# ZhangYuef/Alink

Hardware: AMD Instinct MI355X
Metric: rows/sec/node + iters-to-converge, KMeans k=100 1e8-row×128-dim at 1/2/4/8 MI355X (higher is better)
Workload: dtype bf16

## Files before the change

alink_amd/ops/csrc/kmeans_v10.hip:

```cpp
#include <hip/hip_runtime.h>
#include <stdint.h>
#include <stdlib.h>

#ifndef KM10_TIMING
#define KM10_TIMING 0
#endif

#ifndef KM10_PFD
#define KM10_PFD 0
#endif

#include "kmeans_tile.h"
#include "kmeans_v10_body.h"

namespace {

using namespace kmtile;

typedef float f32x32 __attribute__((ext_vector_type(32)));
typedef float f32x16 __attribute__((ext_vector_type(16)));
typedef float f32x4v __attribute__((ext_vector_type(4)));
typedef uint32_t u32x4 __attribute__((ext_vector_type(4)));

enum Mode10 { FULL = 0, LOAD_ONLY = 1, COMPUTE_ONLY = 2, DIST_ONLY = 3, ACC_ONLY = 4 };

constexpr int NBUF = 9;
constexpr int AHEAD = 7;
constexpr int OFF_ASG = NBUF * TILE;
constexpr uint32_t IDX_MODE = 0xC000u;
constexpr int OFF_CNT = OFF_ASG + 512;
constexpr int OFF_DYN = OFF_CNT + 128 * 4;
constexpr int OFF_JUNK = OFF_DYN + 8 * 4;
constexpr int LDS_BYTES = OFF_JUNK + 256;
constexpr int CH = 16;
constexpr int RED_STRIDE = 112 * D;
static_assert(LDS_BYTES <= LDS_CAP && 2 * RED_STRIDE * 4 <= NBUF * TILE, "LDS plan");


__device__ __forceinline__ float max3_raw(float a, float b, float c) {
    float r;
    asm("v_max3_f32 %0, %1, %2, %3" : "=v"(r) : "v"(a), "v"(b), "v"(c));
    return r;
}
__device__ __forceinline__ float max_raw(float a, float b) {
    float r;
    asm("v_max_f32 %0, %1, %2" : "=v"(r) : "v"(a), "v"(b));
    return r;
}

template <int NT>
__device__ __forceinline__ void dma_tile(uint32_t m0v, uint32_t voff, __amdgpu_buffer_rsrc_t rs, uint32_t soff) {
    uint32_t keep, m1, s1, s2, s3;
#define KM10_DMA(POL)                                                                                       \
    asm volatile(                                                                                           \
        "s_mov_b32 %0, m0\n\t"                                                                              \
        "s_mov_b32 m0, %7\n\t"                                                                              \
        "s_add_u32 %2, %8, 4096\n\t"                                                                        \
        "buffer_load_dwordx4 %5, %6, %8 offen " POL " lds\n\t"                                              \
        "s_add_u32 %1, %7, 4096\n\t"                                                                        \
        "s_mov_b32 m0, %1\n\t"                                                                              \
        "s_add_u32 %3, %8, 8192\n\t"                                                                        \
        "buffer_load_dwordx4 %5, %6, %2 offen " POL " lds\n\t"                                              \
        "s_add_u32 %1, %7, 8192\n\t"                                                                        \
        "s_mov_b32 m0, %1\n\t"                                                                              \
        "s_add_u32 %4, %8, 12288\n\t"                                                                       \
        "buffer_load_dwordx4 %5, %6, %3 offen " POL " lds\n\t"                                              \
        "s_add_u32 %1, %7, 12288\n\t"                                                                       \
        "s_mov_b32 m0, %1\n\t"                                                                              \
        "s_nop 0\n\t"                                                                                       \
        "buffer_load_dwordx4 %5, %6, %4 offen " POL " lds\n\t"                                              \
        "s_mov_b32 m0, %0"                                                                                  \
        : "=&s"(keep), "=&s"(m1), "=&s"(s1), "=&s"(s2), "=&s"(s3)                                           \
        : "v"(voff), "s"(rs), "s"(m0v), "s"(soff)                                                           \
        : "memory")
    if constexpr (NT) KM10_DMA("nt");
    else KM10_DMA("");
#undef KM10_DMA
}

__device__ __forceinline__ void l2_touch(uint32_t m0v, uint32_t voff, __amdgpu_buffer_rsrc_t rs, uint32_t soff) {
    uint32_t keep;
    asm volatile(
        "s_mov_b32 %0, m0\n\t"
        "s_mov_b32 m0, %3\n\t"
        "s_nop 0\n\t"
        "buffer_load_dword %1, %2, %4 offen lds\n\t"
        "s_mov_b32 m0, %0"
        : "=&s"(keep)
        : "v"(voff), "s"(rs), "s"(m0v), "s"(soff)
        : "memory");
}

template <int KB, int MODE, int NT, int DYN>
__global__ __launch_bounds__(512) void kmeans_v10_kernel(const __bf16* __restrict__ Xp, int64_t N,
                                                         const __bf16* __restrict__ Cp,
                                                         const float* __restrict__ ninit, float* __restrict__ slab,
                                                         float* __restrict__ slab_cnt, int* __restrict__ assign_out,
                                                         int64_t ntiles, int64_t per, int rev,
                                                         unsigned* __restrict__ dyn_ctr, int dyn_par, int nqs,
                                                         int64_t pool_base, int npool,
                                                         const unsigned* __restrict__ skip, int pfd_arg) {
    static_assert(KB >= 1 && KB <= 7, "v10 holds at most 112 centroids in registers");
    const int pfd = KM10_PFD ? pfd_arg : 0;
    constexpr bool LOADS = MODE == FULL || MODE == LOAD_ONLY;
    __shared__ __attribute__((aligned(1024))) char lds[LDS_BYTES];
    if (skip != nullptr && __hip_atomic_load(skip, __ATOMIC_RELAXED, __HIP_MEMORY_SCOPE_AGENT) != 0u) return;
    const int tid = threadIdx.x;
    const int lane = tid & 63;
    const int wave = __builtin_amdgcn_readfirstlane(tid >> 6);
    const int g = lane >> 4;
    const int li = lane & 15;
    const int64_t tbase = (int64_t)blockIdx.x * per;
    const int nt = (int)(ntiles > tbase ? (ntiles - tbase < per ? ntiles - tbase : per) : 0);
    const int np = (nt + 1) >> 1;
    const int ntp = 2 * np;
    const uint32_t lbase = (uint32_t)(uintptr_t)(LDS_AS void*)lds;
#if KM10_TIMING
    int64_t* const stamp = reinterpret_cast<int64_t*>(assign_out) + 16 * (int64_t)blockIdx.x;
    if (tid == 0) stamp[0] = (int64_t)__builtin_amdgcn_s_memrealtime();
    assign_out = nullptr;
#endif
    auto phys = [&](int t) { return rev ? ntp - 1 - t : t; };
    int* const dstate = reinterpret_cast<int*>(lds + OFF_DYN);
    int* const qbase = dstate + 4;
    auto dphys = [&](int t) -> int64_t {
        const int q = t / CH, o = t % CH;
        if (q < nqs) {
            const int qq = rev ? nqs - 1 - q : q;
            return ((int64_t)blockIdx.x * nqs + qq) * CH + (rev ? CH - 1 - o : o);
        }
        return (int64_t)qbase[q & 3] + o;
    };

    const bool dma_wave = wave >= 4;
    const int prow = (tid & 255) >> 4;
    const uint32_t voff = (uint32_t)(prow * ROWB + (((tid & 15)) ^ xsw(prow)) * 16);
    const int64_t rem_rows = N - tbase * TR;
    const int64_t region = rem_rows * ROWB < (int64_t)nt * TILE ? rem_rows * ROWB : (int64_t)nt * TILE;
    const __amdgpu_buffer_rsrc_t rs = __builtin_amdgcn_make_buffer_rsrc(
        (void*)(reinterpret_cast<const char*>(Xp) + tbase * TILE), (short)0, (int)(region > 0 ? region : 0),
        0x00020000);
    const uint32_t m0_wave = lbase + (uint32_t)((wave - 4) * 1024);
    const uint32_t pf_off = (uint32_t)((wave - 4) * 4096 + lane * 64);
    uint32_t stage_slot = 0;
    auto next_slot = [](uint32_t s) { return s == (uint32_t)((NBUF - 1) * TILE) ? 0u : s + (uint32_t)TILE; };
    auto stage_tile = [&](int t) {
        if constexpr (DYN) {
            const int64_t pt = __builtin_amdgcn_readfirstlane((int)dphys(t));
            const int64_t remb = (N - pt * TR) * ROWB;
            const __amdgpu_buffer_rsrc_t rt = __builtin_amdgcn_make_buffer_rsrc(
                (void*)(reinterpret_cast<const char*>(Xp) + pt * TILE), (short)0,
                (int)(remb <= 0 ? 0 : (remb < TILE ? remb : TILE)), 0x00020000);
            dma_tile<NT>(__builtin_amdgcn_readfirstlane(m0_wave + (uint32_t)(t % NBUF) * TILE), voff, rt, 0u);
        } else {
            dma_tile<NT>(__builtin_amdgcn_readfirstlane(m0_wave + stage_slot), voff, rs,
                         __builtin_amdgcn_readfirstlane((uint32_t)phys(t) * TILE));
            stage_slot = next_slot(stage_slot);
            if (pfd > 0) {
                const int pt = t + pfd < ntp ? t + pfd : ntp - 1;
                l2_touch(lbase + OFF_JUNK, pf_off, rs, __builtin_amdgcn_readfirstlane((uint32_t)phys(pt) * TILE));
            }
        }
    };
    int last_staged = -1;
    if constexpr (DYN) {
        if (tid == 0) {
            if (blockIdx.x == 0) dyn_ctr[dyn_par ^ 1] = 0u;
            int nq = nqs, done = npool <= 0;
            while (!done && nq * CH < AHEAD) {
                const unsigned r = __hip_atomic_fetch_add(dyn_ctr + dyn_par, 1u, __ATOMIC_RELAXED,
                                                          __HIP_MEMORY_SCOPE_AGENT);
                if ((int)r < npool) {
                    qbase[nq & 3] = (int)(pool_base + (int64_t)(rev ? npool - 1 - (int)r : (int)r) * CH);
                    ++nq;
                } else {
                    done = 1;
                }
            }
            dstate[0] = nq;
            dstate[1] = done;
        }
        __syncthreads();
        if (LOADS && dma_wave) {
            const int known = dstate[0] * CH;
            for (int s = 0; s < AHEAD; ++s)
                if (s < known) {
                    stage_tile(s);
                    last_staged = s;
                }
        }
    } else {
        if (LOADS && dma_wave)
            for (int s = 0; s < AHEAD - 2; ++s)
                if (s < ntp) stage_tile(s);
    }
    uint32_t* cnt = reinterpret_cast<uint32_t*>(lds + OFF_CNT);
    if (tid < 128) cnt[tid] = 0u;
    if (tid < 128) reinterpret_cast<uint32_t*>(lds + OFF_ASG)[tid] = IDX_MODE | (IDX_MODE << 16);
#if KM10_TIMING
    uint64_t wait_vm_cyc = 0, wait_bar_cyc = 0;
#endif
    int np_dyn = 0x3fffffff;
    auto read_state = [&](int j) {
        const int nq = dstate[2 * (j & 1)], done = dstate[2 * (j & 1) + 1];
        np_dyn = done ? nq * CH / 2 : 0x3fffffff;
        return nq;
    };

    auto pre = [&](int j) {
        if constexpr (DYN) {
            if (LOADS && dma_wave) {
                const int younger = last_staged - (2 * j + 1);
                if (younger >= 3) wait_vm<12>();
                else if (younger == 2) wait_vm<8>();
                else if (younger == 1) wait_vm<4>();
                else wait_vm<0>();
            }
            barrier_lds();
            const int known = read_state(j) * CH;
            if (LOADS && dma_wave) {
                if (2 * j + AHEAD - 2 < known) {
                    stage_tile(2 * j + AHEAD - 2);
                    last_staged = 2 * j + AHEAD - 2;
                }
                if (2 * j + AHEAD - 1 < known) {
                    stage_tile(2 * j + AHEAD - 1);
                    last_staged = 2 * j + AHEAD - 1;
                }
            }
            return;
        }
#if KM10_TIMING
        const uint64_t tw0 = __builtin_readcyclecounter();
#endif
        if (LOADS && dma_wave && j < np) {
            const int issued = 2 * j + AHEAD - 3 < ntp - 1 ? 2 * j + AHEAD - 3 : ntp - 1;
            const int younger = issued - (2 * j + 1);
            if (pfd > 0) {
                if (younger >= 3) wait_vm<16>();
                else if (younger == 2) wait_vm<11>();
                else if (younger == 1) wait_vm<6>();
                else wait_vm<1>();
            } else {
                wait_tile_np<4, 3>(younger);
            }
        }
#if KM10_TIMING
        const uint64_t tw1 = __builtin_readcyclecounter();
#endif
        barrier_lds();
#if KM10_TIMING
        wait_vm_cyc += tw1 - tw0;
        wait_bar_cyc += __builtin_readcyclecounter() - tw1;
#endif
        if (LOADS && dma_wave) {
            if (2 * j + AHEAD - 2 < ntp) stage_tile(2 * j + AHEAD - 2);
            if (2 * j + AHEAD - 1 < ntp) stage_tile(2 * j + AHEAD - 1);
        }
    };

    if (wave < 4) {
        const int myrow = 16 * wave + li;
        const int apos = 16 * ((myrow >> 2) & 3) + 4 * (myrow >> 4) + (myrow & 3);
        bf16x8 cf[KB][4];
        f32x4 nin[KB];
#pragma unroll
        for (int b = 0; b < KB; ++b) {
#pragma unroll
            for (int s = 0; s < 4; ++s)
                cf[b][s] = *reinterpret_cast<const bf16x8*>(Cp + (16 * b + li) * D + 8 * (s + 4 * g));
            nin[b] = *reinterpret_cast<const f32x4*>(ninit + 16 * b + 4 * g);
        }
        int xr[4];
#pragma unroll
        for (int s = 0; s < 4; ++s) xr[s] = xoff(myrow, s + 4 * g);
        auto load_frag = [&](uint32_t slot, bf16x8 (&x)[4]) {
            const char* xt = lds + slot;
#pragma unroll
            for (int s = 0; s < 4; ++s) x[s] = *reinterpret_cast<const bf16x8*>(xt + xr[s]);
        };
        auto cross_max = [&](float run) {
            const uint32_t u = __float_as_uint(run);
            const auto p32 = __builtin_amdgcn_permlane32_swap(u, u, false, false);
            const uint32_t u2 = __float_as_uint(max_raw(__uint_as_float(p32[0]), __uint_as_float(p32[1])));
            const auto p16 = __builtin_amdgcn_permlane16_swap(u2, u2, false, false);
            return __float_as_uint(max_raw(__uint_as_float(p16[0]), __uint_as_float(p16[1])));
        };
        uint32_t keepmask;
        asm volatile("v_mov_b32 %0, 0xffffff80" : "=v"(keepmask));
        const uint32_t g4 = 4u * (uint32_t)g;
        auto packs = [&](float v, uint32_t field) { return __uint_as_float((__float_as_uint(v) & keepmask) | field); };
        auto rare_neg = [&](const bf16x8 (&x)[4], uint32_t u, uint32_t c) {
            float run = -3.4e38f;
#pragma unroll
            for (int b = 0; b < KB; ++b) {
                f32x4 acc = nin[b];
#pragma unroll
                for (int s = 0; s < 4; ++s) acc = __builtin_amdgcn_mfma_f32_16x16x32_bf16(cf[b][s], x[s], acc, 0, 0, 0);
                const uint32_t c0 = (uint32_t)(16 * b);
                run = max3_raw(run, packs(acc[0], c0), packs(acc[1], c0 + 1));
                run = max3_raw(run, packs(acc[2], c0 + 2), packs(acc[3], c0 + 3));
            }
            const uint32_t v = cross_max(__uint_as_float(__float_as_uint(run) + g4));
            return (int32_t)u < 0 ? (v & 127u) : c;
        };
        auto pair_max = [&](const bf16x8 (&xa_)[4], const bf16x8 (&xb_)[4], uint32_t& ca, uint32_t& cb) {
            f32x4 acc[2 * KB];
            float run[2] = {-3.4e38f, -3.4e38f};
            float p0 = 0.f, p1 = 0.f, p2 = 0.f, p3 = 0.f;
            uint32_t uA = 0u, w0 = 0u, w1 = 0u;
            auto seam = [&](int i) {
                if (i == 0) {
                    uA = __float_as_uint(run[0]) - g4;
                    const auto p32 = __builtin_amdgcn_permlane32_swap(uA, uA, false, false);
                    w0 = p32[0];
                    w1 = p32[1];
                } else if (i == 1) {
                    const uint32_t u2 = __float_as_uint(max_raw(__uint_as_float(w0), __uint_as_float(w1)));
                    const auto p16 = __builtin_amdgcn_permlane16_swap(u2, u2, false, false);
                    w0 = p16[0];
                    w1 = p16[1];
                } else {
                    uA = __float_as_uint(max_raw(__uint_as_float(w0), __uint_as_float(w1)));
                }
            };
#pragma unroll
            for (int t = 0; t < 2 * KB + 2; ++t) {
                const bool mf = t < 2 * KB, vl = t >= 2;
                const int b = t < KB ? t : t - KB;
                const int pt = (t - 2) / KB, pb = (t - 2) % KB;
                const uint32_t f0 = 127u - (uint32_t)(16 * pb);
                auto mfma = [&](int s) {
                    if (!mf) return;
                    acc[t] = __builtin_amdgcn_mfma_f32_16x16x32_bf16(cf[b][s], t < KB ? xa_[s] : xb_[s],
                                                                     s == 0 ? nin[b] : acc[t], 0, 0, 0);
                };
                mfma(0);
                if (vl) {
                    p0 = packs(acc[t - 2][0], f0);
                    p1 = packs(acc[t - 2][1], f0 - 1);
                }
                __builtin_amdgcn_sched_barrier(0);
                mfma(1);
                if (vl) {
                    run[pt] = max3_raw(run[pt], p0, p1);
                    p2 = packs(acc[t - 2][2], f0 - 2);
                }
                __builtin_amdgcn_sched_barrier(0);
                mfma(2);
                if (vl) {
                    p3 = packs(acc[t - 2][3], f0 - 3);
                    run[pt] = max3_raw(run[pt], p2, p3);
                }
                __builtin_amdgcn_sched_barrier(0);
                mfma(3);
                if (mf && t >= KB + 2 && t < KB + 5) seam(t - KB - 2);
                __builtin_amdgcn_sched_barrier(0);
            }
#pragma unroll
            for (int i = 0; i < 3; ++i)
                if (KB + 2 + i >= 2 * KB) seam(i);
            const uint32_t uB = cross_max(__uint_as_float(__float_as_uint(run[1]) - g4));
            ca = 127u - (uA & 127u);
            cb = 127u - (uB & 127u);
            if (__builtin_amdgcn_ballot_w64((int32_t)(uA | uB) < 0) != 0) {
                ca = rare_neg(xa_, uA, ca);
                cb = rare_neg(xb_, uB, cb);
            }
        };
        const int64_t row_end = DYN ? N : ((tbase + nt) * TR < N ? (tbase + nt) * TR : N);
        auto publish = [&](int j, int h, uint32_t c) {
            if (g == 0) {
                const int64_t grow = (DYN ? dphys(2 * j + h) : tbase + phys(2 * j + h)) * TR + myrow;
                reinterpret_cast<uint16_t*>(lds + OFF_ASG)[(j & 1) * 128 + h * 64 + apos] =
                    (uint16_t)(IDX_MODE | (2 * c));
                if (grow < row_end) {
                    __hip_atomic_fetch_add(cnt + c, 1u, __ATOMIC_RELAXED, __HIP_MEMORY_SCOPE_WORKGROUP);
                    if (assign_out != nullptr) assign_out[grow] = (int)c;
                }
            }
        };
        bf16x8 xa[4], xb[4];
        int pend = 0;
        unsigned pend_v = 0u;
        uint32_t slot_a = 0;
#if KM10_TIMING
        const uint64_t loop0 = __builtin_readcyclecounter();
#endif
        for (int j = 0; DYN || j <= np; ++j) {
            pre(j);
            if constexpr (DYN) {
                if (j > np_dyn) break;
                if (wave == 0) {
                    int nq = dstate[2 * (j & 1)], done = dstate[2 * (j & 1) + 1];
                    if (pend) {
                        const unsigned r = __builtin_amdgcn_readfirstlane(pend_v);
                        if ((int)r < npool) {
                            if (lane == 0)
                                qbase[nq & 3] = (int)(pool_base + (int64_t)(rev ? npool - 1 - (int)r : (int)r) * CH);
                            ++nq;
                        } else {
                            done = 1;
                        }
                        pend = 0;
                    }
                    if (!done && nq <= (2 * j + 2 * AHEAD - 4) / CH) {
                        if (lane == 0)
                            pend_v = __hip_atomic_fetch_add(dyn_ctr + dyn_par, 1u, __ATOMIC_RELAXED,
                                                            __HIP_MEMORY_SCOPE_AGENT);
                        pend = 1;
                    }
                    if (lane == 0) {
                        dstate[2 * ((j + 1) & 1)] = nq;
                        dstate[2 * ((j + 1) & 1) + 1] = done;
                    }
                }
            }
            const int npj = DYN ? np_dyn : np;
            if (MODE == LOAD_ONLY || MODE == ACC_ONLY || j >= npj) continue;
            const uint32_t slot_b = next_slot(slot_a);
            load_frag(slot_a, xa);
            load_frag(slot_b, xb);
            slot_a = next_slot(slot_b);
            uint32_t c0, c1;
            pair_max(xa, xb, c0, c1);
            publish(j, 0, c0);
            publish(j, 1, c1);
#if KM10_TIMING
            if (j == 0 && tid == 0) stamp[1] = (int64_t)__builtin_amdgcn_s_memrealtime();
#endif
        }
#if KM10_TIMING
        if (tid == 0) {
            stamp[2] = (int64_t)__builtin_amdgcn_s_memrealtime();
            stamp[8] = (int64_t)wait_vm_cyc;
            stamp[9] = (int64_t)wait_bar_cyc;
            stamp[10] = (int64_t)(__builtin_readcyclecounter() - loop0);
        }
#endif
        barrier_lds();
        barrier_lds();
        barrier_lds();
    } else {
        const int a = wave - 4;
        const uint32_t aoff =
            lbase + (uint32_t)(a * 1024) + ((uint32_t)(16 * (lane >> 2) + 4 * (lane & 3)) ^ (uint32_t)(a << 4));
        f32x32 s0 = {}, s1 = {}, s2 = {}, s3 = {}, s4 = {}, s5 = {}, s6 = {};
        f32x16 xv = {};
        auto acc_tile = [&](uint32_t slot, const u32x4& v0, const u32x4& v1) {
            const uint32_t w0 = __builtin_amdgcn_readfirstlane(v0[0]), w1 = __builtin_amdgcn_readfirstlane(v0[1]);
            const uint32_t w2 = __builtin_amdgcn_readfirstlane(v0[2]), w3 = __builtin_amdgcn_readfirstlane(v0[3]);
            const uint32_t w4 = __builtin_amdgcn_readfirstlane(v1[0]), w5 = __builtin_amdgcn_readfirstlane(v1[1]);
            const uint32_t w6 = __builtin_amdgcn_readfirstlane(v1[2]), w7 = __builtin_amdgcn_readfirstlane(v1[3]);
            const uint32_t base = aoff + slot;
            f32x4v addr;
            uint32_t keep;
            asm volatile(KM10_ACC_BODY
                         : "+{v[32:63]}"(s0), "+{v[64:95]}"(s1), "+{v[96:127]}"(s2), "+{v[128:159]}"(s3),
                           "+{v[160:191]}"(s4), "+{v[192:223]}"(s5), "+{v[224:255]}"(s6), "+{v[16:31]}"(xv),
                           "=&{v[12:15]}"(addr), [keep] "=&s"(keep)
                         : [base] "v"(base), [w0] "s"(w0), [w1] "s"(w1), [w2] "s"(w2), [w3] "s"(w3), [w4] "s"(w4),
                           [w5] "s"(w5), [w6] "s"(w6), [w7] "s"(w7), [one_lo] "s"(0x3F80u),
                           [one_hi] "s"(0x3F800000u)
                         : "memory");
        };
        uint32_t slot_a = 0;
        __builtin_amdgcn_s_setprio(1);
#if KM10_TIMING
        const uint64_t loop0 = __builtin_readcyclecounter();
#endif
        for (int j = 0; DYN || j <= np; ++j) {
            pre(j);
            if (DYN && j > np_dyn) break;
            if (MODE == LOAD_ONLY || MODE == DIST_ONLY || j == 0) continue;
            const char* ab = lds + OFF_ASG + ((j - 1) & 1) * 256 + 32 * a;
            const u32x4 a0 = *reinterpret_cast<const u32x4*>(ab), a1 = *reinterpret_cast<const u32x4*>(ab + 16);
            const u32x4 b0 = *reinterpret_cast<const u32x4*>(ab + 128), b1 = *reinterpret_cast<const u32x4*>(ab + 144);
            const uint32_t slot_b = next_slot(slot_a);
            acc_tile(slot_a, a0, a1);
            acc_tile(slot_b, b0, b1);
            slot_a = next_slot(slot_b);
        }
        if (LOADS && pfd > 0) wait_vm<0>();
#if KM10_TIMING
        if (tid == 256) {
            stamp[3] = (int64_t)__builtin_amdgcn_s_memrealtime();
            stamp[11] = (int64_t)wait_vm_cyc;
            stamp[12] = (int64_t)wait_bar_cyc;
            stamp[13] = (int64_t)(__builtin_readcyclecounter() - loop0);
        }
#endif
        barrier_lds();
        float* R = reinterpret_cast<float*>(lds) + (a & 1) * RED_STRIDE;
        const f32x32 sv[7] = {s0, s1, s2, s3, s4, s5, s6};
        if (MODE != LOAD_ONLY && a < 2) {
#pragma unroll
            for (int b = 0; b < KB; ++b)
#pragma unroll
                for (int e = 0; e < 16; ++e) {
                    R[(16 * b + e) * D + 2 * lane] = sv[b][2 * e];
                    R[(16 * b + e) * D + 2 * lane + 1] = sv[b][2 * e + 1];
                }
        }
        barrier_lds();
        if (MODE != LOAD_ONLY && a >= 2) {
#pragma unroll
            for (int b = 0; b < KB; ++b)
#pragma unroll
                for (int e = 0; e < 16; ++e) {
                    R[(16 * b + e) * D + 2 * lane] += sv[b][2 * e];
                    R[(16 * b + e) * D + 2 * lane + 1] += sv[b][2 * e + 1];
                }
        }
        barrier_lds();
    }
#if KM10_TIMING
    if (tid == 0) stamp[4] = (int64_t)__builtin_amdgcn_s_memrealtime();
#endif
    if (MODE != LOAD_ONLY) {
        const float* R0 = reinterpret_cast<const float*>(lds);
        float* S = slab + (int64_t)blockIdx.x * 128 * D;
        for (int e = tid * 4; e < 16 * KB * D; e += 512 * 4) {
            const f32x4v u = *reinterpret_cast<const f32x4v*>(R0 + e);
            const f32x4v v = *reinterpret_cast<const f32x4v*>(R0 + RED_STRIDE + e);
            *reinterpret_cast<f32x4v*>(S + e) = u + v;
        }
        if (tid < 128) slab_cnt[(int64_t)blockIdx.x * 128 + tid] = tid < 16 * KB ? (float)cnt[tid] : 0.f;
    }
#if KM10_TIMING
    if (tid == 0) {
        stamp[5] = (int64_t)__builtin_amdgcn_s_memrealtime();
        stamp[6] = 0;
        stamp[7] = 0;
    }
#endif
}

struct DynArgs {
    unsigned* ctr = nullptr;
    int par = 0;
    int nqs = 0;
    int64_t pool_base = 0;
    int npool = 0;
    const unsigned* skip = nullptr;
    int pfd = 0;
};

template <int KB, int NT>
hipError_t launch10(int mode, dim3 grid, hipStream_t st, const __bf16* X, int64_t N, const __bf16* C,
                    const float* ninit, float* slab, float* slab_cnt, int* assign_out, int64_t ntiles, int64_t per,
                    int rev, const DynArgs& dy) {
#define KM10_ARGS X, N, C, ninit, slab, slab_cnt, assign_out, ntiles, per, rev, dy.ctr, dy.par, dy.nqs, dy.pool_base, \
                  dy.npool, dy.skip, dy.ctr != nullptr ? 0 : dy.pfd
    if (dy.ctr != nullptr) {
        if (mode != FULL) return hipErrorInvalidValue;
        hipLaunchKernelGGL((kmeans_v10_kernel<KB, FULL, NT, 1>), grid, dim3(512), 0, st, KM10_ARGS);
        return hipGetLastError();
    }
    if (mode == DIST_ONLY || mode == ACC_ONLY) {
        if constexpr (KB == 7) {
            if (mode == DIST_ONLY)
                hipLaunchKernelGGL((kmeans_v10_kernel<KB, DIST_ONLY, NT, 0>), grid, dim3(512), 0, st, KM10_ARGS);
            else
                hipLaunchKernelGGL((kmeans_v10_kernel<KB, ACC_ONLY, NT, 0>), grid, dim3(512), 0, st, KM10_ARGS);
            return hipGetLastError();
        }
        return hipErrorInvalidValue;
    }
    if (mode == LOAD_ONLY)
        hipLaunchKernelGGL((kmeans_v10_kernel<KB, LOAD_ONLY, NT, 0>), grid, dim3(512), 0, st, KM10_ARGS);
    else if (mode == COMPUTE_ONLY)
        hipLaunchKernelGGL((kmeans_v10_kernel<KB, COMPUTE_ONLY, NT, 0>), grid, dim3(512), 0, st, KM10_ARGS);
    else
        hipLaunchKernelGGL((kmeans_v10_kernel<KB, FULL, NT, 0>), grid, dim3(512), 0, st, KM10_ARGS);
#undef KM10_ARGS
    return hipGetLastError();
}

template <int KB>
hipError_t launch10_kb(int mode, dim3 grid, hipStream_t st, const __bf16* X, int64_t N, const __bf16* C,
                       const float* ninit, float* slab, float* slab_cnt, int* assign_out, int64_t ntiles,
                       int64_t per, const DynArgs& dy) {
    const bool cached = (mode >> 4) & 1;
    const int rev = (mode >> 5) & 1;
    const int m = mode & 7;
    return cached ? launch10<KB, 0>(m, grid, st, X, N, C, ninit, slab, slab_cnt, assign_out, ntiles, per, rev, dy)
                  : launch10<KB, 1>(m, grid, st, X, N, C, ninit, slab, slab_cnt, assign_out, ntiles, per, rev, dy);
}

}

extern "C" {

int alink_kmeans_assign_accum_bf16_v10(const void* X, int64_t N, const void* C, const float* ninit, int k,
                                       float* slab, float* slab_cnt, int grid, void* stream, int* assign_out,
                                       int mode, const void* skip, void* ctr_v, int par, double pool_frac) {
    unsigned* ctr = reinterpret_cast<unsigned*>(ctr_v);
    if (N <= 0 || k < 1 || k > 112 || grid <= 0) return -1;
    const int KB = (k + 15) / 16;
    const int64_t ntiles = (N + TR - 1) / TR;
    if (grid > ntiles) grid = (int)ntiles;
    const int64_t per = (ntiles + grid - 1) / grid;
    if (per * TILE >= ((int64_t)1 << 31)) return -1;
    int g2 = (int)((ntiles + per - 1) / per);
    DynArgs dy;
    dy.skip = reinterpret_cast<const unsigned*>(skip);
#if KM10_PFD
    {
        const char* e = getenv("ALINK_KMEANS_V10_PFD");
        dy.pfd = e != nullptr ? atoi(e) : 0;
        if (dy.pfd < 0 || dy.pfd > 64) dy.pfd = 0;
    }
#endif
    if (ctr != nullptr) {
        if (skip != nullptr) return -1;
        if (ntiles >= ((int64_t)1 << 31) || pool_frac < 0.0 || pool_frac > 1.0) return -1;
        g2 = grid;
        dy.ctr = ctr;
        dy.par = par & 1;
        dy.nqs = (int)((double)ntiles * (1.0 - pool_frac) / ((double)grid * CH));
        dy.pool_base = (int64_t)grid * dy.nqs * CH;
        dy.npool = (int)((ntiles - dy.pool_base + CH - 1) / CH);
    }
    hipStream_t st = reinterpret_cast<hipStream_t>(stream);
    const __bf16* Xb = (const __bf16*)X;
    const __bf16* Cb = (const __bf16*)C;
    hipError_t e;
    switch (KB) {
        case 1: e = launch10_kb<1>(mode, dim3(g2), st, Xb, N, Cb, ninit, slab, slab_cnt, assign_out, ntiles, per, dy); break;
        case 2: e = launch10_kb<2>(mode, dim3(g2), st, Xb, N, Cb, ninit, slab, slab_cnt, assign_out, ntiles, per, dy); break;
        case 3: e = launch10_kb<3>(mode, dim3(g2), st, Xb, N, Cb, ninit, slab, slab_cnt, assign_out, ntiles, per, dy); break;
        case 4: e = launch10_kb<4>(mode, dim3(g2), st, Xb, N, Cb, ninit, slab, slab_cnt, assign_out, ntiles, per, dy); break;
        case 5: e = launch10_kb<5>(mode, dim3(g2), st, Xb, N, Cb, ninit, slab, slab_cnt, assign_out, ntiles, per, dy); break;
        case 6: e = launch10_kb<6>(mode, dim3(g2), st, Xb, N, Cb, ninit, slab, slab_cnt, assign_out, ntiles, per, dy); break;
        default: e = launch10_kb<7>(mode, dim3(g2), st, Xb, N, Cb, ninit, slab, slab_cnt, assign_out, ntiles, per, dy); break;
    }
    return (int)e;
}

int alink_kmeans_v10_grid(int64_t N, int grid) {
    const int64_t ntiles = (N + TR - 1) / TR;
    if (grid > ntiles) grid = (int)ntiles;
    const int64_t per = (ntiles + grid - 1) / grid;
    return (int)((ntiles + per - 1) / per);
}

}
```

alink_amd/ops/csrc/kmeans_v10_body.h:

```cpp
#pragma once
#define KM10_ACC_BODY \
    "v_mov_b32 v12, %[base]\n\t" \
    "v_xor_b32 v13, 64, %[base]\n\t" \
    "v_xor_b32 v14, 0x80, %[base]\n\t" \
    "v_xor_b32 v15, 0xc0, %[base]\n\t" \
    "s_mov_b32 %[keep], m0\n\t" \
    "ds_read_b32 v16, v12 offset:0\n\t" \
    "ds_read_b32 v17, v13 offset:256\n\t" \
    "ds_read_b32 v18, v14 offset:512\n\t" \
    "ds_read_b32 v19, v15 offset:768\n\t" \
    "ds_read_b32 v20, v12 offset:4096\n\t" \
    "ds_read_b32 v21, v13 offset:4352\n\t" \
    "ds_read_b32 v22, v14 offset:4608\n\t" \
    "ds_read_b32 v23, v15 offset:4864\n\t" \
    "ds_read_b32 v24, v12 offset:8192\n\t" \
    "ds_read_b32 v25, v13 offset:8448\n\t" \
    "ds_read_b32 v26, v14 offset:8704\n\t" \
    "ds_read_b32 v27, v15 offset:8960\n\t" \
    "ds_read_b32 v28, v12 offset:12288\n\t" \
    "ds_read_b32 v29, v13 offset:12544\n\t" \
    "ds_read_b32 v30, v14 offset:12800\n\t" \
    "ds_read_b32 v31, v15 offset:13056\n\t" \
    "s_set_gpr_idx_on %[w0], gpr_idx(SRC2,DST)\n\t" \
    "s_waitcnt lgkmcnt(12)\n\t" \
    "v_dot2_f32_bf16 v32, v16, %[one_lo], v32\n\t" \
    "v_dot2_f32_bf16 v33, v16, %[one_hi], v33\n\t" \
    "s_lshr_b32 m0, %[w0], 16\n\t" \
    "v_dot2_f32_bf16 v32, v17, %[one_lo], v32\n\t" \
    "v_dot2_f32_bf16 v33, v17, %[one_hi], v33\n\t" \
    "s_mov_b32 m0, %[w1]\n\t" \
    "v_dot2_f32_bf16 v32, v18, %[one_lo], v32\n\t" \
    "v_dot2_f32_bf16 v33, v18, %[one_hi], v33\n\t" \
    "s_lshr_b32 m0, %[w1], 16\n\t" \
    "v_dot2_f32_bf16 v32, v19, %[one_lo], v32\n\t" \
    "v_dot2_f32_bf16 v33, v19, %[one_hi], v33\n\t" \
    "s_waitcnt lgkmcnt(8)\n\t" \
    "s_mov_b32 m0, %[w2]\n\t" \
    "v_dot2_f32_bf16 v32, v20, %[one_lo], v32\n\t" \
    "v_dot2_f32_bf16 v33, v20, %[one_hi], v33\n\t" \
    "s_lshr_b32 m0, %[w2], 16\n\t" \
    "v_dot2_f32_bf16 v32, v21, %[one_lo], v32\n\t" \
    "v_dot2_f32_bf16 v33, v21, %[one_hi], v33\n\t" \
    "s_mov_b32 m0, %[w3]\n\t" \
    "v_dot2_f32_bf16 v32, v22, %[one_lo], v32\n\t" \
    "v_dot2_f32_bf16 v33, v22, %[one_hi], v33\n\t" \
    "s_lshr_b32 m0, %[w3], 16\n\t" \
    "v_dot2_f32_bf16 v32, v23, %[one_lo], v32\n\t" \
    "v_dot2_f32_bf16 v33, v23, %[one_hi], v33\n\t" \
    "s_waitcnt lgkmcnt(4)\n\t" \
    "s_mov_b32 m0, %[w4]\n\t" \
    "v_dot2_f32_bf16 v32, v24, %[one_lo], v32\n\t" \
    "v_dot2_f32_bf16 v33, v24, %[one_hi], v33\n\t" \
    "s_lshr_b32 m0, %[w4], 16\n\t" \
    "v_dot2_f32_bf16 v32, v25, %[one_lo], v32\n\t" \
    "v_dot2_f32_bf16 v33, v25, %[one_hi], v33\n\t" \
    "s_mov_b32 m0, %[w5]\n\t" \
    "v_dot2_f32_bf16 v32, v26, %[one_lo], v32\n\t" \
    "v_dot2_f32_bf16 v33, v26, %[one_hi], v33\n\t" \
    "s_lshr_b32 m0, %[w5], 16\n\t" \
    "v_dot2_f32_bf16 v32, v27, %[one_lo], v32\n\t" \
    "v_dot2_f32_bf16 v33, v27, %[one_hi], v33\n\t" \
    "s_waitcnt lgkmcnt(0)\n\t" \
    "s_mov_b32 m0, %[w6]\n\t" \
    "v_dot2_f32_bf16 v32, v28, %[one_lo], v32\n\t" \
    "v_dot2_f32_bf16 v33, v28, %[one_hi], v33\n\t" \
    "s_lshr_b32 m0, %[w6], 16\n\t" \
    "v_dot2_f32_bf16 v32, v29, %[one_lo], v32\n\t" \
    "v_dot2_f32_bf16 v33, v29, %[one_hi], v33\n\t" \
    "s_mov_b32 m0, %[w7]\n\t" \
    "v_dot2_f32_bf16 v32, v30, %[one_lo], v32\n\t" \
    "v_dot2_f32_bf16 v33, v30, %[one_hi], v33\n\t" \
    "s_lshr_b32 m0, %[w7], 16\n\t" \
    "v_dot2_f32_bf16 v32, v31, %[one_lo], v32\n\t" \
    "v_dot2_f32_bf16 v33, v31, %[one_hi], v33\n\t" \
    "s_set_gpr_idx_off\n\t" \
    "s_mov_b32 m0, %[keep]\n\t" \
    ""
```

Before: 24.48 billion.

## Split kmeans v10 loops into steady-state path and fuse paired accumulate asm

The distance and accumulate loops are split into a peeled general iteration, a steady-state body with bounds checks removed (fixed vmcnt wait, unconditional staging, a simplified publish without edge handling), and a general tail. DMA staging offsets now advance incrementally instead of being recomputed from phys(t). The two per-tile accumulate asm blocks are merged into one pair block that reads assignment indices via ds_read plus v_readlane, uses ds_read2st64 to halve LDS read instructions, and overlaps the second tile's reads with the first tile's dot products. The intent is less scalar and branch overhead and better LDS latency hiding, at the cost of hard-coded SGPR clobbers (s83-s99) and more code size.

```diff
diff --git a/alink_amd/ops/csrc/kmeans_v10.hip b/alink_amd/ops/csrc/kmeans_v10.hip
--- a/alink_amd/ops/csrc/kmeans_v10.hip
+++ b/alink_amd/ops/csrc/kmeans_v10.hip
@@ -10,6 +10,8 @@
 #define KM10_PFD 0
 #endif
 
+#include <type_traits>
+
 #include "kmeans_tile.h"
 #include "kmeans_v10_body.h"
 
@@ -20,7 +22,6 @@
 typedef float f32x32 __attribute__((ext_vector_type(32)));
 typedef float f32x16 __attribute__((ext_vector_type(16)));
 typedef float f32x4v __attribute__((ext_vector_type(4)));
-typedef uint32_t u32x4 __attribute__((ext_vector_type(4)));
 
 enum Mode10 { FULL = 0, LOAD_ONLY = 1, COMPUTE_ONLY = 2, DIST_ONLY = 3, ACC_ONLY = 4 };
 
@@ -72,7 +73,7 @@
         "s_mov_b32 m0, %0"                                                                                  \
         : "=&s"(keep), "=&s"(m1), "=&s"(s1), "=&s"(s2), "=&s"(s3)                                           \
         : "v"(voff), "s"(rs), "s"(m0v), "s"(soff)                                                           \
-        : "memory")
+        : "memory", "scc")
     if constexpr (NT) KM10_DMA("nt");
     else KM10_DMA("");
 #undef KM10_DMA
@@ -101,6 +102,9 @@
                                                          int64_t pool_base, int npool,
                                                          const unsigned* __restrict__ skip, int pfd_arg) {
     static_assert(KB >= 1 && KB <= 7, "v10 holds at most 112 centroids in registers");
+    constexpr bool SPLIT = !DYN && !KM10_PFD;
+    using steady_t = std::integral_constant<bool, true>;
+    using general_t = std::integral_constant<bool, false>;
     const int pfd = KM10_PFD ? pfd_arg : 0;
     constexpr bool LOADS = MODE == FULL || MODE == LOAD_ONLY;
     __shared__ __attribute__((aligned(1024))) char lds[LDS_BYTES];
@@ -143,6 +147,8 @@
     const uint32_t m0_wave = lbase + (uint32_t)((wave - 4) * 1024);
     const uint32_t pf_off = (uint32_t)((wave - 4) * 4096 + lane * 64);
     uint32_t stage_slot = 0;
+    uint32_t stage_soff = rev ? (uint32_t)(ntp - 1) * TILE : 0u;
+    const uint32_t stage_step = rev ? 0u - (uint32_t)TILE : (uint32_t)TILE;
     auto next_slot = [](uint32_t s) { return s == (uint32_t)((NBUF - 1) * TILE) ? 0u : s + (uint32_t)TILE; };
     auto stage_tile = [&](int t) {
         if constexpr (DYN) {
@@ -154,8 +160,9 @@
             dma_tile<NT>(__builtin_amdgcn_readfirstlane(m0_wave + (uint32_t)(t % NBUF) * TILE), voff, rt, 0u);
         } else {
             dma_tile<NT>(__builtin_amdgcn_readfirstlane(m0_wave + stage_slot), voff, rs,
-                         __builtin_amdgcn_readfirstlane((uint32_t)phys(t) * TILE));
+                         __builtin_amdgcn_readfirstlane(stage_soff));
             stage_slot = next_slot(stage_slot);
+            stage_soff += stage_step;
             if (pfd > 0) {
                 const int pt = t + pfd < ntp ? t + pfd : ntp - 1;
                 l2_touch(lbase + OFF_JUNK, pf_off, rs, __builtin_amdgcn_readfirstlane((uint32_t)phys(pt) * TILE));
@@ -207,7 +214,8 @@
         return nq;
     };
 
-    auto pre = [&](int j) {
+    auto sync = [&](int j, auto steady) {
+        constexpr bool ST = decltype(steady)::value;
         if constexpr (DYN) {
             if (LOADS && dma_wave) {
                 const int younger = last_staged - (2 * j + 1);
@@ -233,7 +241,9 @@
 #if KM10_TIMING
         const uint64_t tw0 = __builtin_readcyclecounter();
 #endif
-        if (LOADS && dma_wave && j < np) {
+        if constexpr (ST) {
+            if (LOADS && dma_wave) wait_vm<12>();
+        } else if (LOADS && dma_wave && j < np) {
             const int issued = 2 * j + AHEAD - 3 < ntp - 1 ? 2 * j + AHEAD - 3 : ntp - 1;
             const int younger = issued - (2 * j + 1);
             if (pfd > 0) {
@@ -253,9 +263,13 @@
         wait_vm_cyc += tw1 - tw0;
         wait_bar_cyc += __builtin_readcyclecounter() - tw1;
 #endif
-        if (LOADS && dma_wave) {
-            if (2 * j + AHEAD - 2 < ntp) stage_tile(2 * j + AHEAD - 2);
-            if (2 * j + AHEAD - 1 < ntp) stage_tile(2 * j + AHEAD - 1);
+    };
+    auto stage = [&](int j, auto steady) {
+        if constexpr (!DYN) {
+            if (LOADS && dma_wave) {
+                if (decltype(steady)::value || 2 * j + AHEAD - 2 < ntp) stage_tile(2 * j + AHEAD - 2);
+                if (decltype(steady)::value || 2 * j + AHEAD - 1 < ntp) stage_tile(2 * j + AHEAD - 1);
+            }
         }
     };
 
@@ -380,6 +394,19 @@
                 }
             }
         };
+        auto publish_inner = [&](int j, uint32_t c0, uint32_t c1) {
+            if (g == 0) {
+                uint16_t* const asg = reinterpret_cast<uint16_t*>(lds + OFF_ASG) + (j & 1) * 128 + apos;
+                asg[0] = (uint16_t)(IDX_MODE | (2 * c0));
+                asg[64] = (uint16_t)(IDX_MODE | (2 * c1));
+                __hip_atomic_fetch_add(cnt + c0, 1u, __ATOMIC_RELAXED, __HIP_MEMORY_SCOPE_WORKGROUP);
+                __hip_atomic_fetch_add(cnt + c1, 1u, __ATOMIC_RELAXED, __HIP_MEMORY_SCOPE_WORKGROUP);
+                if (assign_out != nullptr) {
+                    (assign_out + (tbase + phys(2 * j)) * TR)[myrow] = (int)c0;
+                    (assign_out + (tbase + phys(2 * j + 1)) * TR)[myrow] = (int)c1;
+                }
+            }
+        };
         bf16x8 xa[4], xb[4];
         int pend = 0;
         unsigned pend_v = 0u;
@@ -387,10 +414,11 @@
 #if KM10_TIMING
         const uint64_t loop0 = __builtin_readcyclecounter();
 #endif
-        for (int j = 0; DYN || j <= np; ++j) {
-            pre(j);
+        auto dist_iter = [&](int j, auto steady) __attribute__((always_inline)) -> bool {
+            constexpr bool ST = decltype(steady)::value;
+            sync(j, steady);
             if constexpr (DYN) {
-                if (j > np_dyn) break;
+                if (j > np_dyn) return false;
                 if (wave == 0) {
                     int nq = dstate[2 * (j & 1)], done = dstate[2 * (j & 1) + 1];
                     if (pend) {
@@ -417,19 +445,31 @@
                 }
             }
             const int npj = DYN ? np_dyn : np;
-            if (MODE == LOAD_ONLY || MODE == ACC_ONLY || j >= npj) continue;
+            if (MODE == LOAD_ONLY || MODE == ACC_ONLY || (!ST && j >= npj)) return true;
             const uint32_t slot_b = next_slot(slot_a);
             load_frag(slot_a, xa);
             load_frag(slot_b, xb);
             slot_a = next_slot(slot_b);
             uint32_t c0, c1;
             pair_max(xa, xb, c0, c1);
-            publish(j, 0, c0);
-            publish(j, 1, c1);
+            if (!DYN && (ST || j != (rev ? 0 : np - 1))) {
+                publish_inner(j, c0, c1);
+            } else {
+                publish(j, 0, c0);
+                publish(j, 1, c1);
+            }
 #if KM10_TIMING
             if (j == 0 && tid == 0) stamp[1] = (int64_t)__builtin_amdgcn_s_memrealtime();
 #endif
-        }
+            return true;
+        };
+        int j = 0;
+        if constexpr (SPLIT) {
+            dist_iter(0, general_t{});
+            for (j = 1; j < np - 3; ++j) dist_iter(j, steady_t{});
+        }
+        for (; DYN || j <= np; ++j)
+            if (!dist_iter(j, general_t{})) break;
 #if KM10_TIMING
         if (tid == 0) {
             stamp[2] = (int64_t)__builtin_amdgcn_s_memrealtime();
@@ -447,40 +487,44 @@
             lbase + (uint32_t)(a * 1024) + ((uint32_t)(16 * (lane >> 2) + 4 * (lane & 3)) ^ (uint32_t)(a << 4));
         f32x32 s0 = {}, s1 = {}, s2 = {}, s3 = {}, s4 = {}, s5 = {}, s6 = {};
         f32x16 xv = {};
-        auto acc_tile = [&](uint32_t slot, const u32x4& v0, const u32x4& v1) {
-            const uint32_t w0 = __builtin_amdgcn_readfirstlane(v0[0]), w1 = __builtin_amdgcn_readfirstlane(v0[1]);
-            const uint32_t w2 = __builtin_amdgcn_readfirstlane(v0[2]), w3 = __builtin_amdgcn_readfirstlane(v0[3]);
-            const uint32_t w4 = __builtin_amdgcn_readfirstlane(v1[0]), w5 = __builtin_amdgcn_readfirstlane(v1[1]);
-            const uint32_t w6 = __builtin_amdgcn_readfirstlane(v1[2]), w7 = __builtin_amdgcn_readfirstlane(v1[3]);
-            const uint32_t base = aoff + slot;
+        uint32_t idad = lbase + (uint32_t)(OFF_ASG + 32 * a + ((lane & 8) ? 128 : 0) + 4 * (lane & 7));
+        auto acc_pair = [&](uint32_t sa, uint32_t sb) {
             f32x4v addr;
-            uint32_t keep;
-            asm volatile(KM10_ACC_BODY
+            uint32_t idv;
+            asm volatile(KM10_ACC_PAIR
                          : "+{v[32:63]}"(s0), "+{v[64:95]}"(s1), "+{v[96:127]}"(s2), "+{v[128:159]}"(s3),
                            "+{v[160:191]}"(s4), "+{v[192:223]}"(s5), "+{v[224:255]}"(s6), "+{v[16:31]}"(xv),
-                           "=&{v[12:15]}"(addr), [keep] "=&s"(keep)
-                         : [base] "v"(base), [w0] "s"(w0), [w1] "s"(w1), [w2] "s"(w2), [w3] "s"(w3), [w4] "s"(w4),
-                           [w5] "s"(w5), [w6] "s"(w6), [w7] "s"(w7), [one_lo] "s"(0x3F80u),
-                           [one_hi] "s"(0x3F800000u)
-                         : "memory");
+                           "=&{v[12:15]}"(addr), [idv] "=&v"(idv)
+                         : [slota] "s"(sa), [slotb] "s"(sb), [aoff] "v"(aoff), [idad] "v"(idad),
+                           [one_lo] "s"(0x3F80u), [one_hi] "s"(0x3F800000u)
+                         : "memory", "scc", KM10_ACC_PAIR_CLOBBERS);
+            idad ^= 256u;
         };
         uint32_t slot_a = 0;
         __builtin_amdgcn_s_setprio(1);
 #if KM10_TIMING
         const uint64_t loop0 = __builtin_readcyclecounter();
 #endif
-        for (int j = 0; DYN || j <= np; ++j) {
-            pre(j);
-            if (DYN && j > np_dyn) break;
-            if (MODE == LOAD_ONLY || MODE == DIST_ONLY || j == 0) continue;
-            const char* ab = lds + OFF_ASG + ((j - 1) & 1) * 256 + 32 * a;
-            const u32x4 a0 = *reinterpret_cast<const u32x4*>(ab), a1 = *reinterpret_cast<const u32x4*>(ab + 16);
-            const u32x4 b0 = *reinterpret_cast<const u32x4*>(ab + 128), b1 = *reinterpret_cast<const u32x4*>(ab + 144);
+        auto acc_iter = [&](int j, auto steady) __attribute__((always_inline)) -> bool {
+            constexpr bool ST = decltype(steady)::value;
+            sync(j, steady);
+            if (DYN && j > np_dyn) return false;
+            const bool work = !(MODE == LOAD_ONLY || MODE == DIST_ONLY) && (ST || j != 0);
             const uint32_t slot_b = next_slot(slot_a);
-            acc_tile(slot_a, a0, a1);
-            acc_tile(slot_b, b0, b1);
-            slot_a = next_slot(slot_b);
-        }
+            stage(j, steady);
+            if (work) {
+                acc_pair(slot_a, slot_b);
+                slot_a = next_slot(slot_b);
+            }
+            return true;
+        };
+        int j = 0;
+        if constexpr (SPLIT) {
+            acc_iter(0, general_t{});
+            for (j = 1; j < np - 3; ++j) acc_iter(j, steady_t{});
+        }
+        for (; DYN || j <= np; ++j)
+            if (!acc_iter(j, general_t{})) break;
         if (LOADS && pfd > 0) wait_vm<0>();
 #if KM10_TIMING
         if (tid == 256) {
diff --git a/alink_amd/ops/csrc/kmeans_v10_body.h b/alink_amd/ops/csrc/kmeans_v10_body.h
--- a/alink_amd/ops/csrc/kmeans_v10_body.h
+++ b/alink_amd/ops/csrc/kmeans_v10_body.h
@@ -1,78 +1,149 @@
 #pragma once
-#define KM10_ACC_BODY \
-    "v_mov_b32 v12, %[base]\n\t" \
-    "v_xor_b32 v13, 64, %[base]\n\t" \
-    "v_xor_b32 v14, 0x80, %[base]\n\t" \
-    "v_xor_b32 v15, 0xc0, %[base]\n\t" \
-    "s_mov_b32 %[keep], m0\n\t" \
-    "ds_read_b32 v16, v12 offset:0\n\t" \
-    "ds_read_b32 v17, v13 offset:256\n\t" \
-    "ds_read_b32 v18, v14 offset:512\n\t" \
-    "ds_read_b32 v19, v15 offset:768\n\t" \
-    "ds_read_b32 v20, v12 offset:4096\n\t" \
-    "ds_read_b32 v21, v13 offset:4352\n\t" \
-    "ds_read_b32 v22, v14 offset:4608\n\t" \
-    "ds_read_b32 v23, v15 offset:4864\n\t" \
-    "ds_read_b32 v24, v12 offset:8192\n\t" \
-    "ds_read_b32 v25, v13 offset:8448\n\t" \
-    "ds_read_b32 v26, v14 offset:8704\n\t" \
-    "ds_read_b32 v27, v15 offset:8960\n\t" \
-    "ds_read_b32 v28, v12 offset:12288\n\t" \
-    "ds_read_b32 v29, v13 offset:12544\n\t" \
-    "ds_read_b32 v30, v14 offset:12800\n\t" \
-    "ds_read_b32 v31, v15 offset:13056\n\t" \
-    "s_set_gpr_idx_on %[w0], gpr_idx(SRC2,DST)\n\t" \
-    "s_waitcnt lgkmcnt(12)\n\t" \
+#define KM10_ACC_PAIR \
+    "ds_read_b32 %[idv], %[idad]\n\t" \
+    "v_add_u32 v12, %[slota], %[aoff]\n\t" \
+    "v_xor_b32 v13, 64, v12\n\t" \
+    "v_xor_b32 v14, 0x80, v12\n\t" \
+    "v_xor_b32 v15, 0xc0, v12\n\t" \
+    "ds_read2st64_b32 v[16:17], v12 offset0:0 offset1:16\n\t" \
+    "ds_read2st64_b32 v[18:19], v13 offset0:1 offset1:17\n\t" \
+    "ds_read2st64_b32 v[20:21], v14 offset0:2 offset1:18\n\t" \
+    "ds_read2st64_b32 v[22:23], v15 offset0:3 offset1:19\n\t" \
+    "ds_read2st64_b32 v[24:25], v12 offset0:32 offset1:48\n\t" \
+    "ds_read2st64_b32 v[26:27], v13 offset0:33 offset1:49\n\t" \
+    "ds_read2st64_b32 v[28:29], v14 offset0:34 offset1:50\n\t" \
+    "ds_read2st64_b32 v[30:31], v15 offset0:35 offset1:51\n\t" \
+    "v_add_u32 v12, %[slotb], %[aoff]\n\t" \
+    "v_xor_b32 v13, 64, v12\n\t" \
+    "v_xor_b32 v14, 0x80, v12\n\t" \
+    "v_xor_b32 v15, 0xc0, v12\n\t" \
+    "s_mov_b32 s83, m0\n\t" \
+    "s_waitcnt lgkmcnt(8)\n\t" \
+    "v_readlane_b32 s84, %[idv], 0\n\t" \
+    "v_readlane_b32 s85, %[idv], 1\n\t" \
+    "v_readlane_b32 s86, %[idv], 2\n\t" \
+    "v_readlane_b32 s87, %[idv], 3\n\t" \
+    "v_readlane_b32 s88, %[idv], 4\n\t" \
+    "v_readlane_b32 s89, %[idv], 5\n\t" \
+    "v_readlane_b32 s90, %[idv], 6\n\t" \
+    "v_readlane_b32 s91, %[idv], 7\n\t" \
+    "v_readlane_b32 s92, %[idv], 8\n\t" \
+    "v_readlane_b32 s93, %[idv], 9\n\t" \
+    "v_readlane_b32 s94, %[idv], 10\n\t" \
+    "v_readlane_b32 s95, %[idv], 11\n\t" \
+    "v_readlane_b32 s96, %[idv], 12\n\t" \
+    "v_readlane_b32 s97, %[idv], 13\n\t" \
+    "v_readlane_b32 s98, %[idv], 14\n\t" \
+    "v_readlane_b32 s99, %[idv], 15\n\t" \
+    "s_set_gpr_idx_on s84, gpr_idx(SRC2,DST)\n\t" \
+    "s_waitcnt lgkmcnt(4)\n\t" \
     "v_dot2_f32_bf16 v32, v16, %[one_lo], v32\n\t" \
     "v_dot2_f32_bf16 v33, v16, %[one_hi], v33\n\t" \
-    "s_lshr_b32 m0, %[w0], 16\n\t" \
+    "s_lshr_b32 m0, s84, 16\n\t" \
+    "v_dot2_f32_bf16 v32, v18, %[one_lo], v32\n\t" \
+    "v_dot2_f32_bf16 v33, v18, %[one_hi], v33\n\t" \
+    "s_mov_b32 m0, s85\n\t" \
+    "v_dot2_f32_bf16 v32, v20, %[one_lo], v32\n\t" \
+    "v_dot2_f32_bf16 v33, v20, %[one_hi], v33\n\t" \
+    "s_lshr_b32 m0, s85, 16\n\t" \
+    "v_dot2_f32_bf16 v32, v22, %[one_lo], v32\n\t" \
+    "v_dot2_f32_bf16 v33, v22, %[one_hi], v33\n\t" \
+    "s_mov_b32 m0, s86\n\t" \
     "v_dot2_f32_bf16 v32, v17, %[one_lo], v32\n\t" \
     "v_dot2_f32_bf16 v33, v17, %[one_hi], v33\n\t" \
-    "s_mov_b32 m0, %[w1]\n\t" \
+    "s_lshr_b32 m0, s86, 16\n\t" \
+    "v_dot2_f32_bf16 v32, v19, %[one_lo], v32\n\t" \
+    "v_dot2_f32_bf16 v33, v19, %[one_hi], v33\n\t" \
+    "s_mov_b32 m0, s87\n\t" \
+    "v_dot2_f32_bf16 v32, v21, %[one_lo], v32\n\t" \
+    "v_dot2_f32_bf16 v33, v21, %[one_hi], v33\n\t" \
+    "s_lshr_b32 m0, s87, 16\n\t" \
+    "v_dot2_f32_bf16 v32, v23, %[one_lo], v32\n\t" \
+    "v_dot2_f32_bf16 v33, v23, %[one_hi], v33\n\t" \
+    "ds_read2st64_b32 v[16:17], v12 offset0:0 offset1:16\n\t" \
+    "ds_read2st64_b32 v[18:19], v13 offset0:1 offset1:17\n\t" \
+    "ds_read2st64_b32 v[20:21], v14 offset0:2 offset1:18\n\t" \
+    "ds_read2st64_b32 v[22:23], v15 offset0:3 offset1:19\n\t" \
+    "s_waitcnt lgkmcnt(4)\n\t" \
+    "s_mov_b32 m0, s88\n\t" \
+    "v_dot2_f32_bf16 v32, v24, %[one_lo], v32\n\t" \
+    "v_dot2_f32_bf16 v33, v24, %[one_hi], v33\n\t" \
+    "s_lshr_b32 m0, s88, 16\n\t" \
+    "v_dot2_f32_bf16 v32, v26, %[one_lo], v32\n\t" \
+    "v_dot2_f32_bf16 v33, v26, %[one_hi], v33\n\t" \
+    "s_mov_b32 m0, s89\n\t" \
+    "v_dot2_f32_bf16 v32, v28, %[one_lo], v32\n\t" \
+    "v_dot2_f32_bf16 v33, v28, %[one_hi], v33\n\t" \
+    "s_lshr_b32 m0, s89, 16\n\t" \
+    "v_dot2_f32_bf16 v32, v30, %[one_lo], v32\n\t" \
+    "v_dot2_f32_bf16 v33, v30, %[one_hi], v33\n\t" \
+    "s_mov_b32 m0, s90\n\t" \
+    "v_dot2_f32_bf16 v32, v25, %[one_lo], v32\n\t" \
+    "v_dot2_f32_bf16 v33, v25, %[one_hi], v33\n\t" \
+    "s_lshr_b32 m0, s90, 16\n\t" \
+    "v_dot2_f32_bf16 v32, v27, %[one_lo], v32\n\t" \
+    "v_dot2_f32_bf16 v33, v27, %[one_hi], v33\n\t" \
+    "s_mov_b32 m0, s91\n\t" \
+    "v_dot2_f32_bf16 v32, v29, %[one_lo], v32\n\t" \
+    "v_dot2_f32_bf16 v33, v29, %[one_hi], v33\n\t" \
+    "s_lshr_b32 m0, s91, 16\n\t" \
+    "v_dot2_f32_bf16 v32, v31, %[one_lo], v32\n\t" \
+    "v_dot2_f32_bf16 v33, v31, %[one_hi], v33\n\t" \
+    "ds_read2st64_b32 v[24:25], v12 offset0:32 offset1:48\n\t" \
+    "ds_read2st64_b32 v[26:27], v13 offset0:33 offset1:49\n\t" \
+    "ds_read2st64_b32 v[28:29], v14 offset0:34 offset1:50\n\t" \
+    "ds_read2st64_b32 v[30:31], v15 offset0:35 offset1:51\n\t" \
+    "s_waitcnt lgkmcnt(4)\n\t" \
+    "s_mov_b32 m0, s92\n\t" \
+    "v_dot2_f32_bf16 v32, v16, %[one_lo], v32\n\t" \
+    "v_dot2_f32_bf16 v33, v16, %[one_hi], v33\n\t" \
+    "s_lshr_b32 m0, s92, 16\n\t" \
     "v_dot2_f32_bf16 v32, v18, %[one_lo], v32\n\t" \
     "v_dot2_f32_bf16 v33, v18, %[one_hi], v33\n\t" \
-    "s_lshr_b32 m0, %[w1], 16\n\t" \
+    "s_mov_b32 m0, s93\n\t" \
+    "v_dot2_f32_bf16 v32, v20, %[one_lo], v32\n\t" \
+    "v_dot2_f32_bf16 v33, v20, %[one_hi], v33\n\t" \
+    "s_lshr_b32 m0, s93, 16\n\t" \
+    "v_dot2_f32_bf16 v32, v22, %[one_lo], v32\n\t" \
+    "v_dot2_f32_bf16 v33, v22, %[one_hi], v33\n\t" \
+    "s_mov_b32 m0, s94\n\t" \
+    "v_dot2_f32_bf16 v32, v17, %[one_lo], v32\n\t" \
+    "v_dot2_f32_bf16 v33, v17, %[one_hi], v33\n\t" \
+    "s_lshr_b32 m0, s94, 16\n\t" \
     "v_dot2_f32_bf16 v32, v19, %[one_lo], v32\n\t" \
     "v_dot2_f32_bf16 v33, v19, %[one_hi], v33\n\t" \
-    "s_waitcnt lgkmcnt(8)\n\t" \
-    "s_mov_b32 m0, %[w2]\n\t" \
-    "v_dot2_f32_bf16 v32, v20, %[one_lo], v32\n\t" \
-    "v_dot2_f32_bf16 v33, v20, %[one_hi], v33\n\t" \
-    "s_lshr_b32 m0, %[w2], 16\n\t" \
+    "s_mov_b32 m0, s95\n\t" \
     "v_dot2_f32_bf16 v32, v21, %[one_lo], v32\n\t" \
     "v_dot2_f32_bf16 v33, v21, %[one_hi], v33\n\t" \
-    "s_mov_b32 m0, %[w3]\n\t" \
-    "v_dot2_f32_bf16 v32, v22, %[one_lo], v32\n\t" \
-    "v_dot2_f32_bf16 v33, v22, %[one_hi], v33\n\t" \
-    "s_lshr_b32 m0, %[w3], 16\n\t" \
+    "s_lshr_b32 m0, s95, 16\n\t" \
     "v_dot2_f32_bf16 v32, v23, %[one_lo], v32\n\t" \
     "v_dot2_f32_bf16 v33, v23, %[one_hi], v33\n\t" \
-    "s_waitcnt lgkmcnt(4)\n\t" \
-    "s_mov_b32 m0, %[w4]\n\t" \
+    "s_waitcnt lgkmcnt(0)\n\t" \
+    "s_mov_b32 m0, s96\n\t" \
     "v_dot2_f32_bf16 v32, v24, %[one_lo], v32\n\t" \
     "v_dot2_f32_bf16 v33, v24, %[one_hi], v33\n\t" \
-    "s_lshr_b32 m0, %[w4], 16\n\t" \
+    "s_lshr_b32 m0, s96, 16\n\t" \
+    "v_dot2_f32_bf16 v32, v26, %[one_lo], v32\n\t" \
+    "v_dot2_f32_bf16 v33, v26, %[one_hi], v33\n\t" \
+    "s_mov_b32 m0, s97\n\t" \
+    "v_dot2_f32_bf16 v32, v28, %[one_lo], v32\n\t" \
+    "v_dot2_f32_bf16 v33, v28, %[one_hi], v33\n\t" \
+    "s_lshr_b32 m0, s97, 16\n\t" \
+    "v_dot2_f32_bf16 v32, v30, %[one_lo], v32\n\t" \
+    "v_dot2_f32_bf16 v33, v30, %[one_hi], v33\n\t" \
+    "s_mov_b32 m0, s98\n\t" \
     "v_dot2_f32_bf16 v32, v25, %[one_lo], v32\n\t" \
     "v_dot2_f32_bf16 v33, v25, %[one_hi], v33\n\t" \
-    "s_mov_b32 m0, %[w5]\n\t" \
-    "v_dot2_f32_bf16 v32, v26, %[one_lo], v32\n\t" \
-    "v_dot2_f32_bf16 v33, v26, %[one_hi], v33\n\t" \
-    "s_lshr_b32 m0, %[w5], 16\n\t" \
+    "s_lshr_b32 m0, s98, 16\n\t" \
     "v_dot2_f32_bf16 v32, v27, %[one_lo], v32\n\t" \
     "v_dot2_f32_bf16 v33, v27, %[one_hi], v33\n\t" \
-    "s_waitcnt lgkmcnt(0)\n\t" \
-    "s_mov_b32 m0, %[w6]\n\t" \
-    "v_dot2_f32_bf16 v32, v28, %[one_lo], v32\n\t" \
-    "v_dot2_f32_bf16 v33, v28, %[one_hi], v33\n\t" \
-    "s_lshr_b32 m0, %[w6], 16\n\t" \
+    "s_mov_b32 m0, s99\n\t" \
     "v_dot2_f32_bf16 v32, v29, %[one_lo], v32\n\t" \
     "v_dot2_f32_bf16 v33, v29, %[one_hi], v33\n\t" \
-    "s_mov_b32 m0, %[w7]\n\t" \
-    "v_dot2_f32_bf16 v32, v30, %[one_lo], v32\n\t" \
-    "v_dot2_f32_bf16 v33, v30, %[one_hi], v33\n\t" \
-    "s_lshr_b32 m0, %[w7], 16\n\t" \
+    "s_lshr_b32 m0, s99, 16\n\t" \
     "v_dot2_f32_bf16 v32, v31, %[one_lo], v32\n\t" \
     "v_dot2_f32_bf16 v33, v31, %[one_hi], v33\n\t" \
     "s_set_gpr_idx_off\n\t" \
-    "s_mov_b32 m0, %[keep]\n\t" \
+    "s_mov_b32 m0, s83\n\t" \
     ""
+#define KM10_ACC_PAIR_CLOBBERS "s84", "s85", "s86", "s87", "s88", "s89", "s90", "s91", "s92", "s93", "s94", "s95", "s96", "s97", "s98", "s99", "s83"
```

Measured after the change: 25.62 billion (median of 6 runs). 1.05x the previous value.
